# hellobertrand/zxc

Measured on NVIDIA H100. Metric: decompress GB/s (uncompressed), higher is better.
Workload: dtype u8

## Files before the change

zxc_b200/csrc/zxc_decode.cuh:

```cuda
#pragma once
#include <cuda_runtime.h>
#include <stdint.h>

#include <type_traits>

#include "zxc_b200.h"
#include "zxc_error.h"

typedef uint8_t u8;
typedef uint32_t u32;
typedef uint64_t u64;
typedef int32_t i32;

#define FULL 0xFFFFFFFFu
#ifndef ZXC_FASTMOD
#define ZXC_FASTMOD 1
#endif
#ifndef ZXC_TAIL_SMEM
#define ZXC_TAIL_SMEM 1
#endif
#ifndef ZXC_ALIGNED_LD
#define ZXC_ALIGNED_LD 1
#endif
#ifndef ZXC_HINTS
// ... 377 lines not shown
                int rc;
                if (enc_lit == 2) {
                    if (lit_comp < 128) return ZXC_ERROR_CORRUPT_DATA;
                    rc = pivco_decode(p_data, p_data + 128, lit_comp - 128, scratch, n_lit, hw, cum, cum_words, lane);
                } else {
                    rc = pivco_decode(dict_huf, p_data, lit_comp, scratch, n_lit, hw, cum, cum_words, lane);
                }
                if (rc != ZXC_OK) return rc;
                __syncwarp();
                S.lit = scratch;
                S.n_lit_avail = n_lit;
            } else {
                S.lit = p_data;
                S.n_lit_avail = 0;
            }
        } else if (enc_lit == 1) {
            if (n_lit > 0) {
                if (n_lit > cap) return ZXC_ERROR_DST_TOO_SMALL;
                if (n_lit > scratch_cap) return ZXC_ERROR_CORRUPT_DATA;
                if (lit_comp > avail) return ZXC_ERROR_CORRUPT_DATA;
                const int rc = rle_expand(p_data, lit_comp, scratch, n_lit, lane);
                if (rc != ZXC_OK) return rc;
                __syncwarp();
                S.lit = scratch;
                S.n_lit_avail = n_lit;
            } else {
                S.lit = p_data;
                S.n_lit_avail = 0;
            }
        } else if (enc_lit == 0) {
            S.lit = p_data;
            S.n_lit_avail = lit_comp;
        } else {
            return ZXC_ERROR_CORRUPT_DATA;
        }
        const u64 sz_off = enc_off ? (u64)n_seq : (u64)n_seq * 2;
        const u64 consumed = (u64)lit_comp + tok_comp + sz_off;
        if (consumed > avail) return ZXC_ERROR_CORRUPT_DATA;
        if (avail - lit_comp < 32) return ZXC_ERROR_CORRUPT_DATA;
        if (enc_tok != 0 && enc_tok != 2) return ZXC_ERROR_CORRUPT_DATA;
        S.tok = p_data + lit_comp;
        S.offs = S.tok + tok_comp;
        if (LEAN && S.lit == scratch) {
            const u32 ts = tok_comp + (u32)sz_off;
            if ((u64)n_lit + ts > scratch_cap + scr_tok_cap(block_cap) + (u32)HUF_WORK_BYTES) return D2_DEFER_STATUS;
            warp_copy(scratch + n_lit, S.tok, ts, lane);
            __syncwarp();
            S.tok = scratch + n_lit;
        } else if (LEAN && S.n_lit_avail == 0) {
            S.lit = S.tok;
        }
        if (!LEAN && enc_tok == 2) {
            if (n_seq == 0 || n_seq > block_cap / 5u + 16u || tok_comp < 128) return ZXC_ERROR_CORRUPT_DATA;
            const int rc = pivco_decode(S.tok, S.tok + 128, tok_comp - 128, tok_buf, n_seq, hw, cum, cum_words, lane);
            if (rc != ZXC_OK) return rc;
            __syncwarp();
            S.tok = tok_buf;
        }
        S.ext = S.offs + (u32)sz_off;
        S.ext_end = avail - (u32)consumed;
    } else {
        if (enc_lit != 0 || enc_tok != 0) return ZXC_ERROR_CORRUPT_DATA;
        const u32 avail = comp - 12;
        const u64 consumed = (u64)n_lit + (u64)n_seq * 4;
        if (consumed > avail) return ZXC_ERROR_CORRUPT_DATA;
        if (avail - n_lit < 32) return ZXC_ERROR_CORRUPT_DATA;
        S.lit = pay + 12;
        S.n_lit_avail = n_lit;
        S.tok = S.lit + n_lit;
        S.ext = S.tok + (size_t)n_seq * 4;
        S.ext_end = avail - (u32)consumed;
    }
    return ZXC_OK;
}

#include "zxc_decode_units.cuh"

struct Window {
    u8* ring;
    u8* out;
    const u8* dict;
    u32 dict_size;
    i32 near_lo;
};

__device__ __forceinline__ u8 window_byte(const Window& w, i32 pos) {
    if (pos >= w.near_lo) return w.ring[(u32)pos & (RING_BYTES - 1)];
    return pos >= 0 ? w.out[pos] : w.dict[(i32)w.dict_size + pos];
}
__device__ __forceinline__ u8 far_byte(const Window& w, i32 pos) {
    return pos >= 0 ? w.out[pos] : w.dict[(i32)w.dict_size + pos];
}

__device__ __forceinline__ void ring_flush(const Window& w, u32& F, u32 target, u32 lane, bool al16) {
    const u32 mask = RING_BYTES - 1;
    if (target <= F) return;
    if (al16) {
        const u32 head_end = min(target, (F + 15u) & ~15u);
        if (F < head_end) {
            const u32 p = F + lane;
            if (p < head_end) w.out[p] = w.ring[p & mask];
            F = head_end;
        }
#if ZXC_BULK_FLUSH
        const u32 nb = (target - F) & ~15u;
        if (nb) {
            if (lane == 0) {
                const u32 r = F & mask, first = min(nb, RING_BYTES - r);
                st_store_fence();
                st_store(w.out + F, smem_addr(w.ring) + r, first);
                if (first < nb) st_store(w.out + F + first, smem_addr(w.ring), nb - first);
                st_store_commit();
            }
            F += nb;
        }
#else
        while (target - F >= 512u) {
            const uint4 v = *reinterpret_cast<const uint4*>(w.ring + ((F + 16u * lane) & mask));
            *reinterpret_cast<uint4*>(w.out + F + 16u * lane) = v;
            F += 512u;
        }
        const u32 units = (target - F) >> 4;
        if (lane < units) {
            const uint4 v = *reinterpret_cast<const uint4*>(w.ring + ((F + 16u * lane) & mask));
            *reinterpret_cast<uint4*>(w.out + F + 16u * lane) = v;
        }
        F += units << 4;
#endif
    }
    for (u32 p = F + lane; p < target; p += 32) w.out[p] = w.ring[p & mask];
    F = target;
}

__device__ __forceinline__ void flush_wait(u32 lane) {
#if ZXC_BULK_FLUSH
    if (lane == 0) st_store_wait();
    __syncwarp();
#else
    (void)lane;
#endif
}

__device__ __forceinline__ void warp_match_to_ring(const Window& w, u32 d, u32 off, u32 n, u32 lane) {
    const u32 mask = RING_BYTES - 1;
    ZXC_STAT(16, d < off);
    if (off >= 32) {
        for (u32 c = 0; c < n; c += 32) {
            const u32 k = c + lane;
            if (k < n) w.ring[(d + k) & mask] = window_byte(w, (i32)(d + k) - (i32)off);
            __syncwarp();
        }
    } else {
        const u32 mine = lane < off ? (u32)window_byte(w, (i32)d - (i32)off + (i32)lane) : 0u;
        ZXC_STAT(15, 1);
#if ZXC_FASTMOD
        const float inv = __fdividef(1.0f, (float)off);
        u32 step = 32u - (u32)(32.0f * inv) * off;
        if (step >= off) step -= off;
        u32 r = lane - (u32)((float)lane * inv) * off;
        if (r >= off) r -= off;
#else
        const u32 step = 32u % off;
        u32 r = lane % off;
#endif
        for (u32 c = 0; c < n; c += 32) {
            const u32 b = __shfl_sync(FULL, mine, r);
            if (c + lane < n) w.ring[(d + c + lane) & mask] = (u8)b;
            r += step;
            if (r >= off) r -= off;
        }
    }
}

__device__ __forceinline__ void warp_match_global(const Window& w, u32 d, u32 off, u32 n, u32 lane) {
    if (off >= 32) {
        for (u32 c = 0; c < n; c += 32) {
            const u32 k = c + lane;
            if (k < n) w.out[d + k] = far_byte(w, (i32)(d + k) - (i32)off);
            __syncwarp();
        }
    } else {
        for (u32 k = lane; k < n; k += 32) w.out[d + k] = far_byte(w, (i32)d - (i32)off + (i32)(k % off));
    }
}

template <int K, int N>
__device__ __forceinline__ void store_ladder(u32 d0, const u32* D, u32 kt) {
    if constexpr (K < N) {
        if ((u32)K < kt) sts32<4 * K>(d0, D[K]);
        store_ladder<K + 1, N>(d0, D, kt);
    }
}

template <int NWORDS>
__device__ __forceinline__ void lane_copy_words2(u32 ring_s, u32 dpos, const u8* sp, u32 n, bool on) {
    if (on) {
        const u32 da = dpos & 3u;
        const u32 e = da + n;
        const u32 kt = e >> 2;
        const u32 tb = e & 3u;
        const u8* bp = sp - da;
        const u32 m = (u32)(reinterpret_cast<uintptr_t>(bp)) & 3u;
        const u32* wp = reinterpret_cast<const u32*>(bp - m);
        const u32 sh = m * 8u;
        const u32 nsrc = kt + (tb ? 1u : 0u) + (m ? 1u : 0u);
        u32 W[NWORDS + 1];
#pragma unroll
        for (int k = 0; k <= NWORDS; k++) W[k] = (u32)k < nsrc ? wp[k] : 0u;
        u32 D[NWORDS];
#pragma unroll
        for (int k = 0; k < NWORDS; k++) D[k] = __funnelshift_r(W[k], W[k + 1], sh);
        const u32 d0 = ring_s + (dpos & (RING_BYTES - 1)) - da;
        if (da == 0 && kt > 0) sts32<0>(d0, D[0]);
        store_ladder<1, NWORDS>(d0, D, kt);
        {
            const u32 e0 = e < 4u ? e : 4u;
            const u32 bm = da ? ((0xFu << da) & (0xFu >> (4u - e0))) : 0u;
            if (bm & 2u) sts8<1>(d0, D[0] >> 8);
            if ((bm & 0xCu) == 0xCu) sts16<2>(d0, D[0] >> 16);
            if ((bm & 0xCu) == 0x4u) sts8<2>(d0, D[0] >> 16);
            if ((bm & 0xCu) == 0x8u) sts8<3>(d0, D[0] >> 24);
        }
        {
            u32 tv = D[0];
#pragma unroll
            for (int k = 1; k < NWORDS; k++)
                if (kt == (u32)k) tv = D[k];
            const u32 tm = (kt > 0u || da == 0u) ? tb : 0u;
            const u32 dt = d0 + 4u * kt;
            if (tm == 1u) sts8<0>(dt, tv);
            if (tm >= 2u) sts16<0>(dt, tv);
            if (tm == 3u) sts8<2>(dt, tv >> 16);
        }
    }
}

__device__ __forceinline__ void balanced_copy_words(u32 ring_s, u32 m_items, u32 my_d, const u8* my_sp, u32 my_n,
                                                    u32 lane) {
    const bool own = (m_items >> lane) & 1u;
    const u32 o_da = my_d & 3u;
    const u32 o_ff = o_da ? 1u : 0u;
    const u32 o_lfe = (o_da + my_n) >> 2;
    const u32 o_tb = (o_da + my_n) & 3u;
    const u32 o_dbyte = ring_s + (my_d & (RING_BYTES - 1));
    if (own && o_da) {
        sts8<0>(o_dbyte, my_sp[0]);
        if (o_da < 3) sts8<1>(o_dbyte, my_sp[1]);
        if (o_da < 2) sts8<2>(o_dbyte, my_sp[2]);
    }
    if (own && o_tb) {
        const u32 t0 = my_n - o_tb;
        sts8<0>(o_dbyte + t0, my_sp[t0]);
        if (o_tb > 1) sts8<1>(o_dbyte + t0, my_sp[t0 + 1]);
        if (o_tb > 2) sts8<2>(o_dbyte + t0, my_sp[t0 + 2]);
    }
    const u32 c = own ? (o_lfe - o_ff + 3u) >> 2 : 0u;
    const u32 incl = warp_incl_scan(c, lane);
    const u32 total = __shfl_sync(FULL, incl, 31);
    const u32 excl = incl - c;
    const u32 pk = (my_d & (RING_BYTES - 1)) | (my_n << 16);
    const unsigned long long my_sp64 = reinterpret_cast<unsigned long long>(my_sp);
    for (u32 base = 0; base < total; base += 32) {
        ZXC_STAT(8, 1);
        const u32 q = base + lane;
        const bool act = q < total;
        u32 lo = 0, hi = 31;
#pragma unroll
        for (int it = 0; it < 5; it++) {
            const u32 mid = (lo + hi) >> 1;
            const u32 v = __shfl_sync(FULL, incl, mid);
            if (v > q) hi = mid;
            else lo = mid + 1;
        }
        const u32 j = lo & 31u;
        const u32 k = q - __shfl_sync(FULL, excl, j);
        const u32 pj = __shfl_sync(FULL, pk, j);
        const u8* sp = reinterpret_cast<const u8*>(__shfl_sync(FULL, my_sp64, j));
        if (act) {
            const u32 da = pj & 3u;
            const u32 n = pj >> 16;
            const u32 lfe = (da + n) >> 2;
            const u32 w0 = (da ? 1u : 0u) + 4u * k;
            const u8* bp = sp - da;
            const u32 m = (u32)(reinterpret_cast<uintptr_t>(bp)) & 3u;
            const u32* wp = reinterpret_cast<const u32*>(bp - m) + w0;
            const u32 dw = ring_s + (pj & 0xFFFFu) - da + 4u * w0;
            const u32 sh = m * 8u;
            const u32 left = lfe - w0;
            const u32 nsrc = left + (m ? 1u : 0u);
            u32 W[5];
#pragma unroll
            for (int i = 0; i < 5; i++) W[i] = (u32)i < nsrc ? wp[i] : 0u;
            sts32<0>(dw, __funnelshift_r(W[0], W[1], sh));
            if (1 < left) sts32<4>(dw, __funnelshift_r(W[1], W[2], sh));
            if (2 < left) sts32<8>(dw, __funnelshift_r(W[2], W[3], sh));
            if (3 < left) sts32<12>(dw, __funnelshift_r(W[3], W[4], sh));
        }
    }
}

#ifndef ZXC_NW
#define ZXC_NW 8
#endif
#define LIT_SHORT (4u * ZXC_NW - 4u)
#define MATCH_SHORT (4u * ZXC_NW - 4u)

__device__ __forceinline__ u32* esc_table(u8* scratch, u32 block_cap) {
    return reinterpret_cast<u32*>(scratch + scr_lit_cap(block_cap) + scr_tok_cap(block_cap) + (u32)HUF_WORK_BYTES);
}

__device__ __forceinline__ void la_issue_words(u32 slot_s, const u8* tk, u32 n_seq, u32 enc_off, u32 nb, u32 lane) {
    if (nb < n_seq) {
        const u32 nt = min(32u, n_seq - nb), ow = enc_off ? 1u : 2u;
        const bool t = lane < LA_OFF / 4u;
        const u8* s = t ? tk + nb : tk + n_seq + ow * nb;
        const u32 n = t ? nt : ow * nt;
        const u32 x = (u32)reinterpret_cast<uintptr_t>(s) & 3u;
        const u32 k = t ? lane : lane - LA_OFF / 4u;
        if (4u * k < x + n) cp_async4(slot_s + 4u * lane, s - x + 4u * k);
    }
}
__device__ __forceinline__ void la_issue_esc(u32 slot_s, u32 n_val, u32 ob, u32 lane, const DecodeParams& P) {
    if (ob + lane < n_val)
        cp_async4(slot_s + LA_ESC + 4u * lane, esc_table(warp_scratch(P, grid_warp_now()), P.block_cap) + ob + lane);
}
__device__ __forceinline__ u32 la_esc(u32 slot_s, u32 k, u32 ob, u32 n_val, const DecodeParams& P) {
    if (k >= n_val) return 0u;
    if (k - ob < 32u) return lds32(slot_s + LA_ESC + 4u * (k - ob));
    return esc_table(warp_scratch(P, grid_warp_now()), P.block_cap)[k];
}

template <bool UNITS, bool GHI, bool HAS_DICT, bool LEAN>
__device__ int decode_lz_block(const u8* pay, u32 comp, u8* out, u32 cap, const u8* dict_in,
                               u32 dict_size_in, const u8* dict_huf, u8* scratch, u32 scratch_cap, u8* ring,
                               u32 lane, const DecodeParams& P) {
    constexpr bool ghi = GHI;
    const u8* dict = HAS_DICT ? dict_in : (const u8*)0;
    const u32 dict_size = HAS_DICT ? dict_size_in : 0u;
    ZXC_TRACE_DECL;
    ZXC_TRACE_ADD(TR_BLOCKS, 1, lane);
    Sections S;
    const int prc = parse_sections<LEAN>(pay, comp, ghi, cap, dict_huf, scratch, scratch_cap, lane, S);
    if (prc != ZXC_OK) return prc;
    const u8* lit = S.lit;
    const u8* tok = S.tok;
    const u8* offs = S.offs;
    const u8* ext = S.ext;
    const u32 ext_end = S.ext_end, n_lit_avail = S.n_lit_avail, n_seq = S.n_seq, enc_off = S.enc_off;

    if (UNITS && cap <= 65536u) {
        u8* tok_buf = scratch + scr_lit_cap(scratch_cap);
        u8* hw_area = tok_buf + scr_tok_cap(scratch_cap);
        const bool scratch_busy = (lit == scratch) || (tok == tok_buf);
        u8* tab = scratch_busy ? hw_area : scratch;
        const u32 tab_bytes = scratch_busy ? (u32)HUF_WORK_BYTES + scr_cum_cap(scratch_cap)
                                           : scr_stride(scratch_cap) - 256u;
        const int r = decode_lz_units(lit, n_lit_avail, tok, offs, ext, ext_end, n_seq, enc_off, ghi, out, cap, dict,
                                      dict_size, tab, tab_bytes, lane);
        if (r != UW_NOT_TAKEN) return r;
    }

    const u32 mask = RING_BYTES - 1;
    const u32 esc = ghi ? 255u : 15u;
    const u32 lt_mask = (1u << lane) - 1u;
    const bool al16 = (reinterpret_cast<uintptr_t>(out) & 15u) == 0;
    Window w;
    w.ring = ring;
    w.out = out;
    w.dict = dict;
    w.dict_size = dict_size;
    w.near_lo = 0;
    const u32 ring_s = smem_addr(ring);
    (void)ring_s;
    constexpr bool LA = la_on<HAS_DICT, LEAN>();
    const u32 slot_s = ring_s + WARP_SMEM_BYTES;
    (void)slot_s;
#define W_RING()                                     \
    do {                                             \
        if constexpr (LEAN) w.ring = ring_at(ring_s); \
    } while (0)
    u32 O = 0, L = 0, F = 0, epos = 0, ring_lo = 0;

    u32* vals = esc_table(scratch, scratch_cap);
    if constexpr (LEAN) {
        if (4ull * ext_end > scr_cum_cap(scratch_cap)) return D2_DEFER_STATUS;
    }
    if constexpr (LA) {
        cp_async_check_idle();
        la_issue_words(slot_s, tok, n_seq, enc_off, 0u, lane);
    }
    const bool use_vals = LEAN || (ext_end != 0u && 4ull * ext_end <= scr_cum_cap(scratch_cap));
    u32 n_val = 0, ord_base = 0;
    if (use_vals && (!LEAN || ext_end != 0u)) {
        const u32 seg = max(4u, (ext_end + 31u) / 32u);
        const u32 nseg = (ext_end + seg - 1u) / seg;
        const u32 lo = lane * seg, hi = min(ext_end, lo + seg);
        u64 inc = lane < nseg ? z2_seg_map(ext, lo, hi, ext_end) : Z2_MAP_ID;
#pragma unroll
        for (int dd = 1; dd < 32; dd <<= 1) {
            const u64 o = __shfl_up_sync(FULL, inc, dd);
            if (lane >= (u32)dd) inc = z2_map_compose(o, inc);
        }
        u64 excl = __shfl_up_sync(FULL, inc, 1);
        if (lane == 0) excl = Z2_MAP_ID;
        n_val = z2_map_cnt(__shfl_sync(FULL, inc, 31), 0);
        if (lane < nseg) {
            const u32 ent = z2_map_exit(excl, 0);
            if (ent != 3u) z2_seg_values(ext, lo, hi, ext_end, ent, z2_map_cnt(excl, 0), vals);
        }
        __syncwarp();
    }
    if constexpr (LA) la_issue_esc(slot_s, n_val, 0u, lane, P);

#if ZXC_STAGE
    const u32 stage_s = smem_addr(ring) + RING_BYTES;
    TokStream::open(stage_s, tok, (ghi ? 4u : 1u) * n_seq, pay + comp, tok >= pay && tok < pay + comp);
    OffStream::open(stage_s, ghi ? tok : offs, ghi ? 0u : (enc_off ? 1u : 2u) * n_seq, pay + comp, !ghi);
#if ZXC_STAGE_LIT
    LitStream::open(stage_s, lit, n_lit_avail, pay + comp, lit >= pay && lit < pay + comp);
#define ST_LIT_CLOSE() LitStream::close(stage_s)
#else
#define ST_LIT_CLOSE() do { } while (0)
#endif
#define ST_CLOSE()                   \
    do {                             \
        TokStream::close(stage_s);   \
        OffStream::close(stage_s);   \
        ST_LIT_CLOSE();              \
    } while (0)
#else
#define ST_CLOSE() do { } while (0)
#define ST_LIT_CLOSE() do { } while (0)
#endif

    ZXC_TRACE_MARK(TR_START, lane);

    u32 base = 0;
    while (base < n_seq) {
        const u32 i = base + lane;
        const bool valid = i < n_seq;
        u32 ll = 0, ml = 0, off = 1;
        if (LEAN && !HAS_DICT && lane < 4u && L + 128u * lane < n_lit_avail) prefetch_l1(lit + L + 128u * lane);
        if constexpr (LA) {
            cp_async_wait_all();
            __syncwarp();
        }
#if ZXC_STAGE
        const u32 tok_w = ghi ? 4u : 1u, off_w = enc_off ? 1u : 2u;
        const u32 tx0 = (u32)(reinterpret_cast<uintptr_t>(tok) & 15u), ox0 = (u32)(reinterpret_cast<uintptr_t>(offs) & 15u);
        const u32 i_end = min(base + 32u, n_seq);
        const StWindow st_t = TokStream::need(stage_s, tok, tx0 + tok_w * base, tx0 + tok_w * i_end, 0u, lane);
        const StWindow st_o = OffStream::need(stage_s, offs, ox0 + off_w * base, ox0 + off_w * i_end, 0u, lane);
        const bool t_st = tx0 + tok_w * i_end <= st_t.hi, o_st = !ghi && ox0 + off_w * i_end <= st_o.hi;
#endif
        if (valid) {
            u32 a, b = 0;
#if ZXC_STAGE
            if (!ghi) {
                a = t_st ? lds8(st_t.ring_s + ((tx0 + i) & (ST_RING - 1u))) : (u32)tok[i];
                if (!o_st) {
                    b = enc_off ? (u32)offs[i] : ld16(offs + 2 * (size_t)i);
                } else if (enc_off) {
                    b = lds8(st_o.ring_s + ((ox0 + i) & (ST_RING - 1u)));
                } else {
                    const u32 x = ox0 + 2u * i;
                    b = (ox0 & 1u) ? (lds8(st_o.ring_s + (x & (ST_RING - 1u))) |
                                      (lds8(st_o.ring_s + ((x + 1u) & (ST_RING - 1u))) << 8))
                                   : lds16(st_o.ring_s + (x & (ST_RING - 1u)));
                }
            } else if (t_st) {
                const u32 x = tx0 + 4u * i;
                if (tx0 & 3u) {
                    a = lds8(st_t.ring_s + (x & (ST_RING - 1u))) | (lds8(st_t.ring_s + ((x + 1u) & (ST_RING - 1u))) << 8) |
                        (lds8(st_t.ring_s + ((x + 2u) & (ST_RING - 1u))) << 16) |
                        (lds8(st_t.ring_s + ((x + 3u) & (ST_RING - 1u))) << 24);
                } else {
                    a = lds32(st_t.ring_s + (x & (ST_RING - 1u)));
                }
            } else {
                a = ld32(tok + 4 * (size_t)i);
            }
#else
            if (!ghi) {
                const u8* tk = tok;
                if constexpr (LEAN) tk = lit + opaque(n_lit_avail);
                if constexpr (LA) {
                    a = lds8(slot_s + ((u32)reinterpret_cast<uintptr_t>(tk + base) & 3u) + lane);
                    const u32 ox = (u32)reinterpret_cast<uintptr_t>(tk + n_seq + (enc_off ? base : 2u * base)) & 3u;
                    const u32 oa = slot_s + LA_OFF + ox + (enc_off ? lane : 2u * lane);
                    if (enc_off) b = lds8(oa);
                    else if (ox & 1u) b = lds8(oa) | (lds8(oa + 1u) << 8);
                    else b = lds16(oa);
                } else {
                    a = tk[i];
#if ZXC_ALIGNED_LD
                    if (LEAN) {
                        const u32 oi = n_seq + (enc_off ? i : 2u * i);
                        if (enc_off) b = (u32)tk[oi];
                        else if ((reinterpret_cast<uintptr_t>(tk) + n_seq) & 1u) b = ld16(tk + oi);
                        else b = (u32)*reinterpret_cast<const unsigned short*>(tk + oi);
                    } else if (enc_off) b = (u32)offs[i];
                    else if (reinterpret_cast<uintptr_t>(offs) & 1u) b = ld16(offs + 2 * (size_t)i);
                    else b = (u32)reinterpret_cast<const unsigned short*>(offs)[i];
#else
                    b = enc_off ? (u32)offs[i] : ld16(offs + 2 * (size_t)i);
#endif
                }
            } else {
#if ZXC_ALIGNED_LD
                a = (reinterpret_cast<uintptr_t>(tok) & 3u) ? ld32(tok + 4 * (size_t)i) : reinterpret_cast<const u32*>(tok)[i];
#else
                a = ld32(tok + 4 * (size_t)i);
#endif
            }
#endif
            if (!ghi) {
                ll = a >> 4;
                ml = a & 15;
                off = b + 1;
            } else {
                ll = a >> 24;
                ml = (a >> 16) & 0xFF;
                off = (a & 0xFFFF) + 1;
            }
        }
        const bool e_ll = valid && ll == esc, e_ml = valid && ml == esc;
        const u32 m_ll = __ballot_sync(FULL, e_ll), m_ml = __ballot_sync(FULL, e_ml);
        ZXC_TRACE_MARK(TR_UNPACK, lane);
        u32 k_esc = 0, epos_end = epos;
        if ((m_ll | m_ml) && use_vals) {
            const u32* vt = vals;
            if constexpr (LEAN) vt = esc_table(warp_scratch(P, grid_warp_now()), P.block_cap);
            u32 k = ord_base + __popc(m_ll & lt_mask) + __popc(m_ml & lt_mask);
            if constexpr (LA) {
                if (e_ll) {
                    ll += la_esc(slot_s, k, ord_base, n_val, P);
                    k++;
                }
                if (e_ml) ml += la_esc(slot_s, k, ord_base, n_val, P);
            } else {
                if (e_ll) {
                    ll += k < n_val ? vt[k] : 0u;
                    k++;
                }
                if (e_ml) ml += k < n_val ? vt[k] : 0u;
            }
        } else if (ZXC_RARE((m_ll | m_ml) != 0)) {
            const u32 ord_ll = __popc(m_ll & lt_mask) + __popc(m_ml & lt_mask);
            k_esc = __popc(m_ll) + __popc(m_ml);
            u32 my_pos = ext_end;
            for (u32 s = 0; s < k_esc; s++) {
                if (s == ord_ll) my_pos = epos_end;
                epos_end = varint_advance(ext, epos_end, ext_end);
            }
            if (e_ll) ll += read_varint(ext, my_pos, ext_end);
            if (e_ml) ml += read_varint(ext, my_pos, ext_end);
        }
        if (valid) ml += 5;
        const u32 tot = ll + ml;
        const u32 s_ll = warp_incl_scan(ll, lane);
        const u32 s_tot = warp_incl_scan(tot, lane);

        const u32 nvalid = min(32u, n_seq - base);
        const u32 m = __popc(__ballot_sync(FULL, valid && s_tot <= RING_LIMIT));
        const u32 lit_start = L + s_ll - ll;
        const u32 out_start = O + s_tot - tot;
        const u32 mdst = out_start + ll;

        if (ZXC_RARE(m == 0)) {
            const u32 g_ll = __shfl_sync(FULL, ll, 0), g_ml = __shfl_sync(FULL, ml, 0),
                      g_off = __shfl_sync(FULL, off, 0);
            ZXC_STAT(9, 1);
            if (L + g_ll > n_lit_avail || (u64)O + g_ll + g_ml > cap) {
                ST_CLOSE();
                return ZXC_ERROR_OVERFLOW;
            }
            if (O + g_ll + dict_size < g_off) {
                ST_CLOSE();
                return ZXC_ERROR_BAD_OFFSET;
            }
            __syncwarp();
            W_RING();
            ring_flush(w, F, O, lane, al16);
            __syncwarp();
            flush_wait(lane);
            warp_copy(out + O, lit + L, g_ll, lane);
            __syncwarp();
            warp_match_global(w, O + g_ll, g_off, g_ml, lane);
            __syncwarp();
            O += g_ll + g_ml;
            L += g_ll;
            F = O;
            ring_lo = O >= 64 ? O - 64 : 0;
            for (u32 p = ring_lo + lane; p < O; p += 32) w.ring[p & mask] = out[p];
            __syncwarp();
            const u32 q = ((m_ll & 1u) ? 1u : 0u) + ((m_ml & 1u) ? 1u : 0u);
            ord_base += q;
            if (!use_vals)
                for (u32 s = 0; s < q; s++) epos = varint_advance(ext, epos, ext_end);
            base += 1;
            if constexpr (LA) {
                la_issue_words(slot_s, lit + opaque(n_lit_avail), n_seq, enc_off, base, lane);
                la_issue_esc(slot_s, n_val, ord_base, lane, P);
            }
            ZXC_TRACE_MARK(TR_GIANT, lane);
            continue;
        }

        ZXC_STAT(10, m < nvalid);
        ZXC_STAT(11, m < nvalid && !use_vals);
        const bool act = lane < m;
        const bool ovf = act && (lit_start + ll > n_lit_avail || out_start + tot > cap);
        const bool bad = act && (mdst + dict_size < off);
        const u32 m_err = __ballot_sync(FULL, ovf || bad);
        if (ZXC_RARE(m_err != 0)) {
            ZXC_STAT(19, 1);
            const int code = ovf ? ZXC_ERROR_OVERFLOW : ZXC_ERROR_BAD_OFFSET;
            ST_CLOSE();
            return __shfl_sync(FULL, code, __ffs(m_err) - 1);
        }
        const u32 T = __shfl_sync(FULL, s_tot, m - 1), TL = __shfl_sync(FULL, s_ll, m - 1);
        if constexpr (LA) {
            const u32 below = m < 32u ? (1u << m) - 1u : FULL;
            ord_base += __popc(m_ll & below) + __popc(m_ml & below);
            base += m;
            la_issue_words(slot_s, lit + opaque(n_lit_avail), n_seq, enc_off, base, lane);
            la_issue_esc(slot_s, n_val, ord_base, lane, P);
        }
#if ZXC_STAGE && ZXC_STAGE_LIT
        const u32 lx0 = (u32)(reinterpret_cast<uintptr_t>(lit) & 15u);
        const StWindow lw = LitStream::need(stage_s, lit, lx0 + L, lx0 + L + TL, 8u, lane);
#endif
        {
            const i32 a = (i32)(O + T) - (i32)RING_BYTES + 32;
            w.near_lo = a > (i32)ring_lo ? a : (i32)ring_lo;
        }

        flush_wait(lane);
        const i32 src_lo = (i32)mdst - (i32)off;
        const i32 src_end = min((i32)mdst, src_lo + (i32)ml);
        const bool near = src_lo >= w.near_lo;
        const u32 si = (u32)src_lo & mask;
        const bool in_dict = src_lo + (i32)ml + 8 <= 0 && (i32)dict_size + src_lo >= 8;
        const bool m_word_ok = ((mdst & mask) + ml + 4 <= RING_BYTES) &&
                               (near ? (si >= 8 && si + ml + 8 <= RING_BYTES)
                                     : (in_dict || (src_lo >= 8 && src_lo + (i32)ml + 4 <= w.near_lo)));
        const bool m_lane_ok = m_word_ok && ml <= MATCH_SHORT && off >= ml;
        const bool m_grp_ok = m_word_ok && !m_lane_ok && off >= ml;
        auto match_src = [&]() -> const u8* {
            return near ? (LEAN ? ring_at(ring_s + si) : ring + si)
                        : (src_lo < 0 ? dict + ((i32)dict_size + src_lo) : out + src_lo);
        };
        const u8* m_sp = LEAN ? nullptr : match_src();
        const bool l_word_ok = (out_start & mask) + ll + 4 <= RING_BYTES;

        const bool m_free = src_end <= (i32)O;
        if (LEAN && !HAS_DICT && act && m_free && !near && src_lo >= 0) {
            const u8* ps = out + src_lo;
            const u8* pe = ps + ml - 1u;
            prefetch_l1(ps);
            if ((reinterpret_cast<uintptr_t>(ps) ^ reinterpret_cast<uintptr_t>(pe)) >> 7) prefetch_l1(pe);
        }
        ZXC_TRACE_ADD(TR_M_RING, __popc(__ballot_sync(FULL, act && near)), lane);
        ZXC_TRACE_ADD(TR_M_GLOBAL, __popc(__ballot_sync(FULL, act && !near && src_lo >= 0)), lane);
        ZXC_TRACE_ADD(TR_M_DICT, __popc(__ballot_sync(FULL, act && !near && src_lo < 0)), lane);
        ZXC_TRACE_ADD(TR_M_SEQ, __popc(__ballot_sync(FULL, act && !m_free)), lane);
        ZXC_TRACE_ADD(TR_BATCHES, 1, lane);
        ZXC_TRACE_MARK(TR_SCAN, lane);
        ZXC_STAT(0, 1);
        ZXC_STAT(1, m);
        bool lit_pass = true;
#pragma unroll 1
        for (;;) {
            bool ready, lok, gok;
            u32 it_d, it_n;
            const u8* it_sp;
            if (lit_pass) {
                ready = act && ll > 0;
                it_d = out_start;
                it_n = ll;
                it_sp = lit + lit_start;
#if ZXC_STAGE && ZXC_STAGE_LIT
                {
                    const u8* sp_s = lit_ptr(lw, lx0 + lit_start, ll);
                    if (sp_s) it_sp = sp_s;
                    ZXC_STAT(13, __popc(__ballot_sync(FULL, ready && sp_s != 0)));
                    ZXC_STAT(14, __popc(__ballot_sync(FULL, ready)));
                }
#endif
                lok = l_word_ok && ll <= LIT_SHORT;
                gok = l_word_ok && ll > LIT_SHORT;
            } else {
                ready = act && m_free;
                it_d = mdst;
                it_n = ml;
                it_sp = LEAN ? match_src() : m_sp;
                lok = m_lane_ok;
                gok = m_grp_ok;
            }
            lane_copy_words2<ZXC_NW>(ring_s, it_d, it_sp, it_n, ready && lok);
            const u32 m_grp = __ballot_sync(FULL, ready && gok);
            ZXC_STAT(2, 1);
            ZXC_STAT(3, __popc(__ballot_sync(FULL, ready && lok)));
            ZXC_STAT(4, __popc(m_grp));
            ZXC_STAT(5, m_grp != 0);
            ZXC_STAT(6, __popc(__ballot_sync(FULL, ready && !lok && !gok)));
            ZXC_STAT(7, __ballot_sync(FULL, ready && lok) != 0);
            ZXC_STAT(17, __popc(__ballot_sync(FULL, !lit_pass && ready && (lok || gok) && src_lo < 0)));
            ZXC_STAT(18, __popc(__ballot_sync(FULL, !lit_pass && ready && !lok && !gok)));
            ZXC_STAT(20, __popc(__ballot_sync(FULL, !lit_pass && ready && (lok || gok) && near)));
            ZXC_STAT(21, __popc(__ballot_sync(FULL, !lit_pass && ready && (lok || gok) && !near && src_lo >= 0)));
            if (m_grp) balanced_copy_words(ring_s, m_grp, it_d, it_sp, it_n, lane);
            u32 m_slow = __ballot_sync(FULL, ready && !lok && !gok);
            while (ZXC_RARE(m_slow != 0)) {
                const int j = __ffs(m_slow) - 1;
                m_slow &= m_slow - 1;
                const u32 d = __shfl_sync(FULL, it_d, j), n = __shfl_sync(FULL, it_n, j);
                const u32 aux = __shfl_sync(FULL, lit_pass ? lit_start : off, j);
                W_RING();
                if (lit_pass) {
                    for (u32 k = lane; k < n; k += 32) w.ring[(d + k) & mask] = lit[aux + k];
                } else {
                    warp_match_to_ring(w, d, aux, n, lane);
                }
            }
            __syncwarp();
            ZXC_TRACE_MARK(lit_pass ? TR_LIT : TR_MATCH, lane);
            if (!lit_pass) break;
            lit_pass = false;
        }
        {
            u32 rest = __ballot_sync(FULL, act && !m_free);
            const u32 my_pk = ml | ((near && off >= ml) ? 0x80000000u : 0u);
            ZXC_STAT(12, __popc(rest));
            while (rest) {
                const int j = __ffs(rest) - 1;
                rest &= rest - 1;
                const u32 d = __shfl_sync(FULL, mdst, j), pk = __shfl_sync(FULL, my_pk, j);
                const u32 n = pk & 0x7FFFFFFFu;
                if (pk >> 31) {
                    const u32 sl = __shfl_sync(FULL, (u32)src_lo, j);
#if ZXC_TAIL_SMEM
                    for (u32 k = lane; k < n; k += 32) sts8<0>(ring_s + ((d + k) & mask), lds8(ring_s + ((sl + k) & mask)));
#else
                    for (u32 k = lane; k < n; k += 32) ring[(d + k) & mask] = ring[(sl + k) & mask];
#endif
                } else {
                    W_RING();
                    warp_match_to_ring(w, d, __shfl_sync(FULL, off, j), n, lane);
                }
                __syncwarp();
            }
        }
        ZXC_TRACE_MARK(TR_TAIL, lane);

        O += T;
        L += TL;
        W_RING();
        ring_flush(w, F, O & ~511u, lane, al16);
        __syncwarp();
        ZXC_TRACE_MARK(TR_FLUSH, lane);

        if constexpr (LA) {
        } else if (m < nvalid) {
            const u32 below = (1u << m) - 1u;
            const u32 q = __popc(m_ll & below) + __popc(m_ml & below);
            ord_base += q;
            if (!use_vals)
                for (u32 s = 0; s < q; s++) epos = varint_advance(ext, epos, ext_end);
            base += m;
        } else {
            ord_base += __popc(m_ll) + __popc(m_ml);
            epos = epos_end;
            base += 32;
        }
    }
    if constexpr (LA) cp_async_wait_all();

    ST_LIT_CLOSE();
    const u32 rem = n_lit_avail - L;
    if (rem > cap - O) return ZXC_ERROR_OVERFLOW;
    W_RING();
#undef W_RING
    ring_flush(w, F, O, lane, al16);
    __syncwarp();
    flush_wait(lane);
    warp_copy(out + O, lit + L, rem, lane);
    ZXC_TRACE_MARK(TR_END, lane);
    return (int)(O + rem);
}

template <bool UNITS, bool HAS_DICT, bool LEAN = false>
__device__ int decode_job(const DecodeParams& P, const zxc_b200_job_t& job, u8* scratch, u8* ring, u32 lane) {
    const u8* blk = P.src + job.src_off;
    u8* out = P.dst + job.dst_off;
    if (job.src_len < 8) return LEAN ? D2_DEFER_STATUS : ZXC_ERROR_SRC_TOO_SMALL;
    const u32 type = blk[0];
    const u32 comp = ld32(blk + 3);
    const bool verify = (P.flags & FLAG_VERIFY) != 0;
    if (LEAN) {
        const bool whole = !verify && (u64)job.src_len >= 8ull + comp;
        const bool take = whole && (type == BT_RAW || (type == BT_GLO && comp >= 12u && blk[8 + 9] == 0 && blk[8 + 8] <= 1));
        if (!take) return D2_DEFER_STATUS;
    }
    if ((u64)job.src_len < 8ull + comp + (verify ? 4u : 0u)) return ZXC_ERROR_SRC_TOO_SMALL;
    const u8* data = blk + 8;
    if constexpr (!LEAN) {
        if (verify && ld32(data + comp) != warp_checksum(data, comp, lane)) return ZXC_ERROR_BAD_CHECKSUM;
    }
    switch (type) {
        case BT_GLO:
            return decode_lz_block<UNITS, false, HAS_DICT, LEAN>(data, comp, out, job.dst_cap, P.dict, P.dict_size,
                                                                 P.dict_huf, scratch, P.block_cap, ring, lane, P);
        case BT_GHI:
            if constexpr (LEAN) return D2_DEFER_STATUS;
            else return decode_lz_block<UNITS, true, HAS_DICT, false>(data, comp, out, job.dst_cap, P.dict, P.dict_size,
                                                                      P.dict_huf, scratch, P.block_cap, ring, lane, P);
        case BT_RAW:
            if (comp > job.dst_cap) return ZXC_ERROR_DST_TOO_SMALL;
            warp_copy(out, data, comp, lane);
            return (int)comp;
        case BT_EOF:
            return ZXC_ERROR_CORRUPT_DATA;
        default:
            return ZXC_ERROR_BAD_BLOCK_TYPE;
    }
}

template <bool UNITS, bool DEFERRED, bool HAS_DICT, bool LEAN>
__global__ void __launch_bounds__(CTA_THREADS, LEAN ? LEAN_CTAS_PER_SM : CTAS_PER_SM) zxc_decode_kernel(const DecodeParams P) {
    extern __shared__ __align__(16) u8 smem[];
    const u32 lane = threadIdx.x & 31;
    const u32 wic = threadIdx.x >> 5;
    const u32 gwarp = blockIdx.x * WARPS_PER_CTA + wic;
    u8* scratch = warp_scratch(P, gwarp);
    u8* ring = smem + (size_t)wic * (la_on<HAS_DICT, LEAN>() ? LEAN_WARP_SMEM_BYTES : WARP_SMEM_BYTES);
#if ZXC_STAGE
    st_init(smem_addr(ring) + RING_BYTES, lane);
#endif
    if (DEFERRED) {
        const u32 n_def = *P.defer_count;
        if (n_def == 0) return;
        if (n_def <= P.defer_cap) {
            for (;;) {
                unsigned long long k = 0;
                if (lane == 0) k = atomicAdd(P.counter, 1ull);
                k = __shfl_sync(FULL, k, 0);
                if (k >= n_def) break;
                const u32 j = P.defer_list[k];
                const zxc_b200_job_t job = P.jobs[j];
                const int r = decode_job<UNITS, HAS_DICT, false>(P, job, scratch, ring, lane);
                flush_wait(lane);
                __syncwarp();
                if (lane == 0) P.status[j] = r;
            }
            return;
        }
        for (;;) {
            unsigned long long b = 0;
            if (lane == 0) b = atomicAdd(P.counter, 32ull);
            b = __shfl_sync(FULL, b, 0);
            if (b >= P.n_jobs) break;
            const unsigned long long jj = b + lane;
            u32 m = __ballot_sync(FULL, jj < P.n_jobs && P.status[jj] == D2_DEFER_STATUS);
            while (m) {
                const unsigned long long j = b + (u32)(__ffs(m) - 1);
                m &= m - 1;
                const zxc_b200_job_t job = P.jobs[j];
                const int r = decode_job<UNITS, HAS_DICT, false>(P, job, scratch, ring, lane);
                flush_wait(lane);
                __syncwarp();
                if (lane == 0) P.status[j] = r;
            }
        }
        return;
    }
    using JobIx = typename std::conditional<LEAN, u32, unsigned long long>::type;
    u32 ring_s = 0;
    if constexpr (LEAN) ring_s = smem_addr(ring);
    for (;;) {
        ZXC_TRACE_DECL;
        unsigned long long c = 0;
        if (lane == 0) c = atomicAdd(P.counter, 1ull);
        const JobIx j = __shfl_sync(FULL, (JobIx)c, 0);
        ZXC_TRACE_MARK(TR_CLAIM, lane);
        if (j >= P.n_jobs) break;
        const zxc_b200_job_t job = P.jobs[j];
        const int r = LEAN ? decode_job<UNITS, HAS_DICT, LEAN>(P, job, warp_scratch(P, grid_warp_now()), ring_at(ring_s), lane)
                           : decode_job<UNITS, HAS_DICT, LEAN>(P, job, scratch, ring, lane);
        flush_wait(lane);
        __syncwarp();
        if (lane == 0) {
            P.status[j] = r;
            if (LEAN && r == D2_DEFER_STATUS) {
                const u32 slot = atomicAdd(P.defer_count, 1u);
                if (slot < P.defer_cap) P.defer_list[slot] = (u32)j;
            }
        }
    }
}

__global__ void zxc_reduce_kernel(const i32* status, const zxc_b200_job_t* jobs, u32 n,
                                  unsigned long long* out ) {
    const u32 i = blockIdx.x * blockDim.x + threadIdx.x;
    unsigned long long bad = ~0ull, sum = 0;
    if (i < n) {
        const i32 s = status[i];
        if (s < 0 || (u32)s != jobs[i].dst_cap) bad = i;
        else sum = (u32)s;
    }
    for (int d = 16; d >= 1; d >>= 1) {
        const unsigned long long ob = __shfl_xor_sync(FULL, bad, d);
        bad = ob < bad ? ob : bad;
        sum += __shfl_xor_sync(FULL, sum, d);
    }
    if ((threadIdx.x & 31) == 0) {
        if (bad != ~0ull) atomicMin(&out[0], bad);
        if (sum) atomicAdd(&out[1], sum);
    }
}
```

Baseline: 456.0.

## Pack warp scans, narrow per-lane copy when warp max fits, drop dict checks

Merges the two warp inclusive scans (literal length and total length) into a single scan over a packed 32-bit value, halving shuffle work per batch. Adds a warp-uniform dispatch that takes a narrower 6-word per-lane copy when the warp's largest item fits, reducing unrolled copy instructions. Makes dictionary checks compile out when there is no dictionary and simplifies the prefetch guard. Also adds an instruction-budget profiling script and per-width stats. The extra reduce_max and code duplication add some cost and register pressure.

```diff
diff --git a/profiles/lean_instr_budget.py b/profiles/lean_instr_budget.py
--- /dev/null
+++ b/profiles/lean_instr_budget.py
@@ -0,0 +1,245 @@
+import argparse
+import ctypes as C
+import os
+import re
+import shutil
+import subprocess
+import sys
+import tempfile
+
+import numpy as np
+
+HERE = os.path.dirname(os.path.dirname(os.path.abspath(__file__)))
+LEAN = "_Z17zxc_decode_kernelILb0ELb0ELb0ELb1EEv12DecodeParams"
+NVCC = os.environ.get("NVCC") or shutil.which("nvcc") or "/usr/local/cuda/bin/nvcc"
+TOOLS = os.path.dirname(os.path.realpath(NVCC))
+
+ST_BATCHES, ST_PASSES, ST_LONG_CALLS, ST_SLOW, ST_BAL_STEPS, ST_GIANT, ST_TAIL = 0, 2, 5, 6, 8, 9, 12
+ST_LIT_WORDS, ST_MATCH_WORDS = 32, 41
+
+
+def compile_cubin(root, out):
+    csrc = os.path.join(root, "zxc_b200", "csrc")
+    cmd = [NVCC, "-O3", "-std=c++17", "-gencode", "arch=compute_90a,code=sm_90a", "-lineinfo",
+           "-I" + os.path.join(root, "include"), "-I" + csrc, "-Xptxas", "-v", "-cubin", "-o", out,
+           os.path.join(csrc, "zxc_gpu.cu")]
+    r = subprocess.run(cmd, stdout=subprocess.PIPE, stderr=subprocess.STDOUT, text=True)
+    if r.returncode != 0:
+        raise SystemExit(r.stdout[-4000:])
+    return r.stdout
+
+
+def ptxas_line(log):
+    lines = log.splitlines()
+    for k, ln in enumerate(lines):
+        if "Compiling entry function '%s'" % LEAN in ln:
+            return " / ".join(s.split("ptxas info    : ")[-1].strip() for s in lines[k + 1:k + 4]
+                              if "bytes stack" in s or "registers" in s)
+    return "?"
+
+
+def lean_sass(cubin):
+    r = subprocess.run([os.path.join(TOOLS, "nvdisasm"), "-gi", "-c", cubin], stdout=subprocess.PIPE,
+                       stderr=subprocess.STDOUT, text=True)
+    if r.returncode != 0:
+        raise SystemExit(r.stdout[-2000:])
+    out, inside, loc, in_loc, label, since_label = [], False, [], False, None, 0
+    for ln in r.stdout.splitlines():
+        if ln.startswith(".text.") or (ln.startswith("\t.section") and ".text." in ln):
+            inside = (".text." + LEAN) in ln
+            continue
+        if not inside:
+            continue
+        if "//## File" in ln:
+            f, n = re.search(r'"([^"]+)", line (\d+)', ln).groups()
+            loc = (loc if in_loc else []) + [(os.path.basename(f), int(n))]
+            in_loc = True
+            continue
+        in_loc = False
+        lm = re.match(r"(\.L_x_\d+):", ln)
+        if lm:
+            label, since_label = lm.group(1), 0
+            continue
+        m = re.match(r"\s*/\*[0-9a-f]{4,}\*/\s+(?:@!?U?P[T0-9]+\s+)?([A-Z][A-Z0-9_.]*)(.*)", ln)
+        if m:
+            if m.group(1) == "BRA" and since_label == 0 and label and "(" + label + ")" in m.group(2):
+                break
+            since_label += 1
+            out.append((m.group(1), loc))
+    if not out:
+        raise SystemExit(f"{LEAN} not found in {cubin}")
+    return out
+
+
+def find(src, pat, start=0):
+    for k in range(start, len(src)):
+        if pat in src[k]:
+            return k + 1
+    raise SystemExit(f"marker not found in zxc_decode.cuh: {pat!r}")
+
+
+def block_end(src, first):
+    depth = 0
+    for k in range(first - 1, len(src)):
+        depth += src[k].count("{") - src[k].count("}")
+        if depth == 0 and "{" in "".join(src[first - 1:k + 1]):
+            return k + 1
+    raise SystemExit("unbalanced braces")
+
+
+def regions(root):
+    src = open(os.path.join(root, "zxc_b200", "csrc", "zxc_decode.cuh")).read().splitlines()
+    fn = find(src, "__device__ int decode_lz_block(")
+    fn_end = block_end(src, find(src, "{", fn - 1))
+    loop = find(src, "while (base < n_seq) {", fn)
+    unpack = find(src, "ZXC_TRACE_MARK(TR_UNPACK", loop)
+    giant = find(src, "if (ZXC_RARE(m == 0)) {", unpack)
+    giant_end = block_end(src, giant)
+    scan = find(src, "ZXC_TRACE_MARK(TR_SCAN", giant_end)
+    slow = find(src, "while (ZXC_RARE(m_slow != 0)) {", scan)
+    slow_end = block_end(src, slow)
+    pass_mark = find(src, "ZXC_TRACE_MARK(lit_pass ? TR_LIT : TR_MATCH", slow_end)
+    pass_end = block_end(src, find(src, "for (;;) {", scan))
+    tail_loop = find(src, "while (rest) {", pass_end)
+    tail_end = block_end(src, tail_loop)
+    tail = find(src, "ZXC_TRACE_MARK(TR_TAIL", tail_end)
+    loop_end = block_end(src, loop)
+    bal = find(src, "__device__ __forceinline__ void balanced_copy_words(")
+    bal_loop = find(src, "for (u32 base = 0; base < total; base += 32) {", bal)
+    bal_end = block_end(src, bal_loop)
+    assert fn < loop < unpack < giant < giant_end < scan < slow < slow_end <= pass_mark <= pass_end < tail_loop
+    assert tail_loop < tail_end < tail < loop_end < fn_end
+    copies = [k + 1 for k in range(scan, pass_end) if "lane_copy_words2<" in src[k]]
+    return dict(fn=(fn, fn_end), loop=(loop, loop_end), unpack=unpack, giant=(giant, giant_end), scan=scan,
+                slow=(slow, slow_end), passes=pass_end, tail_loop=(tail_loop, tail_end), tail=tail,
+                bal=(bal, bal_loop), bal_loop=(bal_loop, bal_end), copies=[(k, src[k - 1].strip()) for k in copies],
+                narrow=int(next((m.group(1) for m in map(re.compile(r"#define ZXC_NW_NARROW (\d+)").search, src) if m),
+                                0)))
+
+
+def classify(loc, R):
+    fn_lo, fn_hi = R["fn"]
+    outer = next((ln for f, ln in loc if f == "zxc_decode.cuh" and fn_lo <= ln <= fn_hi), None)
+    if outer is None:
+        return "job", "kernel, decode_job, parse_sections (per block)"
+    lo, hi = R["loop"]
+    if outer < lo:
+        return "start", "block start (per block)"
+    if outer > hi:
+        return "end", "block end (per block)"
+    if outer <= R["unpack"]:
+        return "unpack", "unpack"
+    if R["giant"][0] <= outer <= R["giant"][1]:
+        return "giant", "giant sequence (per giant)"
+    if outer <= R["scan"]:
+        return "scan", "escapes, scans, validation, classification"
+    if outer <= R["passes"]:
+        if R["slow"][0] <= outer <= R["slow"][1]:
+            return "slow", "slow item byte paths (per slow item)"
+        for ln, _ in R["copies"]:
+            if outer == ln:
+                return "copy@%d" % ln, "per-lane copy, line %d (per pass that takes it)" % ln
+        inner = loc[0][1] if loc and loc[0][0] == "zxc_decode.cuh" else 0
+        if R["bal_loop"][0] <= inner <= R["bal_loop"][1]:
+            return "bal_step", "balanced copy step (per step)"
+        if R["bal"][0] <= inner < R["bal"][1]:
+            return "bal_call", "balanced copy set-up (per call)"
+        return "pass", "pass loop, rest (per pass)"
+    if R["tail_loop"][0] <= outer <= R["tail_loop"][1]:
+        return "tail_item", "sequence-order tail, per match"
+    if outer <= R["tail"]:
+        return "tail", "sequence-order tail, per batch"
+    return "flush", "flush and advance"
+
+
+def emulator_counts(root_here, mib):
+    sys.path.insert(0, os.path.join(root_here, "tests"))
+    import zxc_corpus as zc
+    import zxc_ctypes as z
+    import zxc_simt as zs
+    ref, prod = z.ZxcLib(z.REF_SO), z.ZxcLib(z.PRODUCT_SO)
+    data = zc.silesia_shaped(mib << 20, seed=1)
+    frame = zc.compress_ref_mt(ref, data, level=3, block_size=65536, checksum=0)
+    st, out, oob, _ = zs.decode_frame(prod, frame)
+    assert all(s == 65536 for s in st[:-1]) and np.array_equal(out, data), "emulator decode differs"
+    s = np.array((C.c_uint64 * 64).in_dll(zs.lib(), "simt_stat"), dtype=np.float64)
+    return s, len(st)
+
+
+def budget(sass, R, s, blocks):
+    b = s[ST_BATCHES]
+    per = {"unpack": 1.0, "scan": 1.0, "tail": 1.0, "flush": 1.0, "pass": s[ST_PASSES] / b,
+           "slow": s[ST_SLOW] / b, "giant": s[ST_GIANT] / b, "tail_item": s[ST_TAIL] / b,
+           "bal_step": s[ST_BAL_STEPS] / b, "bal_call": s[ST_LONG_CALLS] / b,
+           "start": blocks / b, "end": blocks / b, "job": blocks / b}
+    nw = R["narrow"]
+    fit = sum(s[base + w] for base in (ST_LIT_WORDS, ST_MATCH_WORDS) for w in range(nw + 1)) / b if nw else 0.0
+    for ln, text in R["copies"]:
+        per["copy@%d" % ln] = fit if "ZXC_NW_NARROW>" in text else s[ST_PASSES] / b - fit
+    static, dyn, names = {}, {}, {}
+    for op, loc in sass:
+        if op == "NOP":
+            continue
+        key, name = classify(loc, R)
+        static[key] = static.get(key, 0) + 1
+        names[key] = name
+    for k, n in static.items():
+        dyn[k] = n * per.get(k, 0.0)
+    return static, dyn, names
+
+
+def main():
+    ap = argparse.ArgumentParser()
+    ap.add_argument("--root", default=HERE, help="project tree whose zxc_gpu.cu is measured (default: this one)")
+    ap.add_argument("--cubin", help="prebuilt cubin of --root's zxc_gpu.cu (as the Makefile builds it)")
+    ap.add_argument("--mib", type=int, default=8, help="MiB of the bench corpus the emulator decodes")
+    args = ap.parse_args()
+    root = os.path.abspath(args.root)
+    with tempfile.TemporaryDirectory(prefix="zxc_budget_") as tmp:
+        cubin, ptx = args.cubin, ""
+        if not cubin:
+            cubin = os.path.join(tmp, "zxc_gpu.cubin")
+            ptx = ptxas_line(compile_cubin(root, cubin))
+        sass = lean_sass(cubin)
+        so = os.path.join(tmp, "libzxc_simt_decode.so")
+        r = subprocess.run(["make", "-s", "-C", os.path.join(HERE, "tests", "simt"), f"CSRC={root}/zxc_b200/csrc",
+                            f"SO={so}", "EXTRA=-I" + os.path.join(root, "include")],
+                           stdout=subprocess.PIPE, stderr=subprocess.STDOUT, text=True)
+        if r.returncode != 0:
+            raise SystemExit(r.stdout[-3000:])
+        os.environ["ZXC_SIMT_SO"] = so
+        s, blocks = emulator_counts(HERE, args.mib)
+    R = regions(root)
+    static, dyn, names = budget(sass, R, s, blocks)
+    b = s[ST_BATCHES]
+    print(f"## {root}: {LEAN}")
+    print(f"{len([1 for op, _ in sass if op != 'NOP'])} SASS instructions (NOP excluded); ptxas: {ptx or 'prebuilt cubin'}")
+    print(f"emulator, {args.mib} MiB bench corpus: {blocks} blocks, {b / blocks:.1f} batches per block, "
+          f"{s[ST_PASSES] / b:.2f} passes, {s[ST_BAL_STEPS] / b:.3f} balanced steps, {s[ST_SLOW] / b:.3f} slow items, "
+          f"{s[ST_TAIL] / b:.2f} tail matches per batch")
+    lit = [s[ST_LIT_WORDS + w] / b for w in range(9)]
+    mat = [s[ST_MATCH_WORDS + w] / b for w in range(9)]
+    print("passes by destination words of the longest per-lane item (0..8): literal "
+          + " ".join(f"{x:.3f}" for x in lit) + "; match " + " ".join(f"{x:.3f}" for x in mat))
+    phases = [("unpack", ["unpack"]), ("escapes + scans + validation + classification", ["scan"]),
+              ("copy passes (literal + free-match)", ["pass", "slow", "bal_step", "bal_call"]
+               + [k for k in static if k.startswith("copy@")]),
+              ("sequence-order tail", ["tail", "tail_item"]), ("flush and advance", ["flush"]),
+              ("giant sequences", ["giant"]), ("block start, end, job (per block, spread over its batches)",
+                                               ["start", "end", "job"])]
+    print("\n| phase | region | static | per batch |")
+    print("|---|---|---|---|")
+    total = 0.0
+    for ph, keys in phases:
+        sub = 0.0
+        for k in keys:
+            if k in static:
+                print(f"| {ph} | {names[k]} | {static[k]} | {dyn[k]:.1f} |")
+                sub += dyn[k]
+        print(f"| **{ph}** | | | **{sub:.1f}** |")
+        total += sub
+    print(f"| **batch total** | | | **{total:.1f}** |")
+
+
+if __name__ == "__main__":
+    main()
diff --git a/zxc_b200/csrc/zxc_decode.cuh b/zxc_b200/csrc/zxc_decode.cuh
--- a/zxc_b200/csrc/zxc_decode.cuh
+++ b/zxc_b200/csrc/zxc_decode.cuh
@@ -703,6 +703,9 @@
 #ifndef ZXC_NW
 #define ZXC_NW 8
 #endif
+#ifndef ZXC_NW_NARROW
+#define ZXC_NW_NARROW 6
+#endif
 #define LIT_SHORT (4u * ZXC_NW - 4u)
 #define MATCH_SHORT (4u * ZXC_NW - 4u)
 
@@ -959,8 +962,10 @@
         }
         if (valid) ml += 5;
         const u32 tot = ll + ml;
-        const u32 s_ll = warp_incl_scan(ll, lane);
-        const u32 s_tot = warp_incl_scan(tot, lane);
+        static_assert(32u * (RING_LIMIT + 1u) + 4u < (1u << 17), "the packed scan's high field must fit 17 bits");
+        const u32 s_pk = warp_incl_scan((min(tot, RING_LIMIT + 1u) << 15) + min(ll, RING_LIMIT + 1u), lane);
+        const u32 s_ll = s_pk & 0x7FFFu;
+        const u32 s_tot = s_pk >> 15;
 
         const u32 nvalid = min(32u, n_seq - base);
         const u32 m = __popc(__ballot_sync(FULL, valid && s_tot <= RING_LIMIT));
@@ -1042,7 +1047,7 @@
         const i32 src_end = min((i32)mdst, src_lo + (i32)ml);
         const bool near = src_lo >= w.near_lo;
         const u32 si = (u32)src_lo & mask;
-        const bool in_dict = src_lo + (i32)ml + 8 <= 0 && (i32)dict_size + src_lo >= 8;
+        const bool in_dict = HAS_DICT && src_lo + (i32)ml + 8 <= 0 && (i32)dict_size + src_lo >= 8;
         const bool m_word_ok = ((mdst & mask) + ml + 4 <= RING_BYTES) &&
                                (near ? (si >= 8 && si + ml + 8 <= RING_BYTES)
                                      : (in_dict || (src_lo >= 8 && src_lo + (i32)ml + 4 <= w.near_lo)));
@@ -1050,13 +1055,13 @@
         const bool m_grp_ok = m_word_ok && !m_lane_ok && off >= ml;
         auto match_src = [&]() -> const u8* {
             return near ? (LEAN ? ring_at(ring_s + si) : ring + si)
-                        : (src_lo < 0 ? dict + ((i32)dict_size + src_lo) : out + src_lo);
+                        : (HAS_DICT && src_lo < 0 ? dict + ((i32)dict_size + src_lo) : out + src_lo);
         };
         const u8* m_sp = LEAN ? nullptr : match_src();
         const bool l_word_ok = (out_start & mask) + ll + 4 <= RING_BYTES;
 
         const bool m_free = src_end <= (i32)O;
-        if (LEAN && !HAS_DICT && act && m_free && !near && src_lo >= 0) {
+        if (LEAN && !HAS_DICT && act && m_free && !near) {
             const u8* ps = out + src_lo;
             const u8* pe = ps + ml - 1u;
             prefetch_l1(ps);
@@ -1099,7 +1104,10 @@
                 lok = m_lane_ok;
                 gok = m_grp_ok;
             }
-            lane_copy_words2<ZXC_NW>(ring_s, it_d, it_sp, it_n, ready && lok);
+            if (LEAN && !HAS_DICT && __reduce_max_sync(FULL, ready && lok ? (it_d & 3u) + it_n : 0u) <= 4u * ZXC_NW_NARROW)
+                lane_copy_words2<ZXC_NW_NARROW>(ring_s, it_d, it_sp, it_n, ready && lok);
+            else
+                lane_copy_words2<ZXC_NW>(ring_s, it_d, it_sp, it_n, ready && lok);
             const u32 m_grp = __ballot_sync(FULL, ready && gok);
             ZXC_STAT(2, 1);
             ZXC_STAT(3, __popc(__ballot_sync(FULL, ready && lok)));
@@ -1111,6 +1119,8 @@
             ZXC_STAT(18, __popc(__ballot_sync(FULL, !lit_pass && ready && !lok && !gok)));
             ZXC_STAT(20, __popc(__ballot_sync(FULL, !lit_pass && ready && (lok || gok) && near)));
             ZXC_STAT(21, __popc(__ballot_sync(FULL, !lit_pass && ready && (lok || gok) && !near && src_lo >= 0)));
+            for (u32 k = 0; k <= ZXC_NW; k++)
+                ZXC_STAT((lit_pass ? 32 : 41) + k, (__reduce_max_sync(FULL, ready && lok ? (it_d & 3u) + it_n : 0u) + 3u) / 4u == k);
             if (m_grp) balanced_copy_words(ring_s, m_grp, it_d, it_sp, it_n, lane);
             u32 m_slow = __ballot_sync(FULL, ready && !lok && !gok);
             while (ZXC_RARE(m_slow != 0)) {
```

Result: faster. 465.4 (median of 6 runs) (+2.1%).
